# data-man-34/HHFM

Measured on AMD Instinct MI355X. Metric: scored (user,ctx,item) triples/sec + HR@10, Frappe-shape, 1/2/4/8 MI355X, higher is better.
Workload: dtype f32; 1 GPU; FM k=64 Frappe-shape per-row scoring (configs[1], HBM-roofline variant: 8M users + 8M items + 12 ctx ids); rows_per_gpu=33554432, fields=5, k=64, table_rows=16777228, table_bytes=4294970368, parallelism=rows sharded x1, no collective

## Files before the change

hhfm_amd/csrc/fm_rows.hip:

```cpp
#include "hhfm_common.h"

namespace hhfm {

#ifndef HHFM_K1_CAP
#define HHFM_K1_CAP 64
#endif
#ifndef HHFM_K1_WMAP
#define HHFM_K1_WMAP 0
#endif
#ifndef HHFM_K1_CTXKO
#define HHFM_K1_CTXKO 0
#endif
#if (HHFM_K1_WMAP || HHFM_K1_CTXKO) && !defined(HHFM_DIAG_BUILD)
#error "K1 knock-out macros give wrong results: diagnostic builds only (-DHHFM_DIAG_BUILD)"
#endif
#ifndef HHFM_K1_U5
#define HHFM_K1_U5 5
#endif
template <int F>
struct RowsPerLane {
  static constexpr int value =
      F <= 3 ? 6 : (F == 4 ? 4 : (F == 5 ? HHFM_K1_U5 : (F <= 8 ? 3 : 2)));
};

template <int F, int U, bool NT = false>
HHFM_DEV void load_ids(int32_t (&id)[U][F], const int32_t* __restrict__ idx,
                       int64_t base, int64_t B, int g, int RPW, int ncols) {
#pragma unroll
  for (int u = 0; u < U; ++u) {
    int64_t row = base + (int64_t)u * RPW + g;
    const int32_t* p = idx + (row < B ? row : 0) * (int64_t)ncols;
#pragma unroll
    for (int f = 0; f < F; ++f) id[u][f] = load_i32<NT>(p + f);
  }
}

template <int F, int LPR, bool BF16, bool HAS_W, int NTM>
__global__ __launch_bounds__(256) void fm_rows_fast(
    const int32_t* __restrict__ idx, int64_t B, const char* __restrict__ E,
    int64_t M, const float* __restrict__ w, float w0, float* __restrict__ out,
    int32_t* __restrict__ status) {
  constexpr int U = RowsPerLane<F>::value;
  constexpr int RPW = kWave / LPR;
  constexpr int RPI = RPW * U;
  constexpr int64_t ROW_BYTES = (int64_t)LPR * 16;
  constexpr bool NT = NTM == 1;
  using C = Chunk<BF16>;

  const int lane = threadIdx.x & (kWave - 1);
  const int sub = lane & (LPR - 1);
  const int g = lane / LPR;
  const int64_t wave = ((int64_t)blockIdx.x * blockDim.x + threadIdx.x) / kWave;
  const int64_t nwave = ((int64_t)gridDim.x * blockDim.x) / kWave;
  const int64_t stride = nwave * RPI;

  int64_t base = wave * RPI;
  int32_t raw[U][F];
  bool bad = false;
  if (base < B) load_ids<F, U, NT>(raw, idx, base, B, g, RPW, F);

  for (; base < B; base += stride) {
    C c[U][F];
    int32_t id[U][F];
#pragma unroll
    for (int u = 0; u < U; ++u)
#pragma unroll
      for (int f = 0; f < F; ++f) {
        id[u][f] = clamp_id(raw[u][f], M);
        bad |= id[u][f] != raw[u][f];
        if (HHFM_K1_CTXKO && f >= 2) {
#pragma unroll
          for (int e = 0; e < C::kElems; ++e) c[u][f].v[e] = 0.f;
        } else if (NTM == 2 && f < 2)
          c[u][f].template load<true>(E + (int64_t)id[u][f] * ROW_BYTES + sub * 16);
        else
          c[u][f].template load<NT>(E + (int64_t)id[u][f] * ROW_BYTES + sub * 16);
      }

    float wv[U];
    if constexpr (HAS_W) {
      constexpr int WPL = (F + LPR - 1) / LPR;
#pragma unroll
      for (int u = 0; u < U; ++u) {
        wv[u] = 0.f;
#pragma unroll
        for (int r = 0; r < WPL; ++r) {
          const int fsel = r * LPR + sub;
          int32_t my = id[u][0];
#pragma unroll
          for (int f = 1; f < F; ++f) my = (fsel == f) ? id[u][f] : my;
          const float wl = HHFM_K1_WMAP == 1   ? w[my & 0x3ffff]
                           : HHFM_K1_WMAP == 2 ? w[(int64_t)my * 32]
                                               : w[my];
          wv[u] += (fsel < F) ? wl : 0.f;
        }
      }
    }

    load_ids<F, U, NT>(raw, idx, base + stride, B, g, RPW, F);

#pragma unroll
    for (int u = 0; u < U; ++u) {
      float t = 0.f;
#pragma unroll
      for (int e = 0; e < C::kElems; ++e) {
        float s = c[u][0].v[e];
        float q = c[u][0].v[e] * c[u][0].v[e];
#pragma unroll
        for (int f = 1; f < F; ++f) {
          s += c[u][f].v[e];
          q += c[u][f].v[e] * c[u][f].v[e];
        }
        t += 0.5f * (s * s - q);
      }
      t = group_sum<LPR>(t);
      float fb = 0.f;
      if constexpr (HAS_W) fb = group_sum<LPR>(wv[u]);
      const int64_t row = base + (int64_t)u * RPW + g;
      if (sub == 0 && row < B) {
        if constexpr (NT) __builtin_nontemporal_store((t + fb) + w0, out + row);
        else out[row] = (t + fb) + w0;
      }
    }
  }
  report_bad_id(status, bad);
}

template <bool BF16>
__global__ __launch_bounds__(256) void fm_rows_generic(
    const int32_t* __restrict__ idx, int64_t B, int F, const char* __restrict__ E,
    int64_t M, int k, const float* __restrict__ w, float w0,
    float* __restrict__ out, int32_t* __restrict__ status) {
  const int lane = threadIdx.x & (kWave - 1);
  const int64_t wave = ((int64_t)blockIdx.x * blockDim.x + threadIdx.x) / kWave;
  const int64_t nwave = ((int64_t)gridDim.x * blockDim.x) / kWave;
  const int esz = BF16 ? 2 : 4;
  bool bad = false;
  for (int64_t row = wave; row < B; row += nwave) {
    const int32_t* p = idx + row * (int64_t)F;
    for (int f = lane; f < F; f += kWave) bad |= clamp_id(p[f], M) != p[f];
    float t = 0.f;
    for (int e = lane; e < k; e += kWave) {
      float s = 0.f, q = 0.f;
      for (int f = 0; f < F; ++f) {
        const char* r = E + (int64_t)clamp_id(p[f], M) * k * esz;
        float v = BF16 ? bf16_to_f32(reinterpret_cast<const uint16_t*>(r)[e])
                       : reinterpret_cast<const float*>(r)[e];
        s += v;
        q += v * v;
      }
      t += 0.5f * (s * s - q);
    }
    t = group_sum<kWave>(t);
    float fb = 0.f;
    if (w != nullptr)
      for (int f = 0; f < F; ++f) fb += w[clamp_id(p[f], M)];
    if (lane == 0) out[row] = (t + fb) + w0;
  }
  report_bad_id(status, bad);
}

template <int F, int LPR, bool BF16>
__global__ __launch_bounds__(256) void hybrid_rows_fast(
    const int32_t* __restrict__ idx, int64_t B, int nctx,
    const char* __restrict__ E, int64_t M, float* __restrict__ out,
    int32_t* __restrict__ status) {
  constexpr int U = RowsPerLane<F>::value;
  constexpr int RPW = kWave / LPR;
  constexpr int RPI = RPW * U;
  constexpr int64_t ROW_BYTES = (int64_t)LPR * 16;
  using C = Chunk<BF16>;

  const int lane = threadIdx.x & (kWave - 1);
  const int sub = lane & (LPR - 1);
  const int g = lane / LPR;
  const int64_t wave = ((int64_t)blockIdx.x * blockDim.x + threadIdx.x) / kWave;
  const int64_t nwave = ((int64_t)gridDim.x * blockDim.x) / kWave;
  const int64_t stride = nwave * RPI;
  const int ctx_end = 2 + nctx;

  int64_t base = wave * RPI;
  int32_t raw[U][F];
  bool bad = false;
  if (base < B) load_ids<F, U>(raw, idx, base, B, g, RPW, F);

  for (; base < B; base += stride) {
    C c[U][F];
    int32_t id[U][F];
#pragma unroll
    for (int u = 0; u < U; ++u)
#pragma unroll
      for (int f = 0; f < F; ++f) {
        id[u][f] = clamp_id(raw[u][f], M);
        bad |= id[u][f] != raw[u][f];
        c[u][f].load(E + (int64_t)id[u][f] * ROW_BYTES + sub * 16);
      }

    load_ids<F, U>(raw, idx, base + stride, B, g, RPW, F);

#pragma unroll
    for (int u = 0; u < U; ++u) {
      float t = 0.f;
#pragma unroll
      for (int e = 0; e < C::kElems; ++e) {
        float ctx = 0.f, tim = 0.f;
#pragma unroll
        for (int f = 2; f < F; ++f) {
          if (f < ctx_end) ctx += c[u][f].v[e];
          else tim += c[u][f].v[e];
        }
        float h = c[u][0].v[e];
        if (nctx > 0) h = h + ctx;
        if (ctx_end < F) h = h + tim;
        t += h * c[u][1].v[e];
      }
      t = group_sum<LPR>(t);
      const int64_t row = base + (int64_t)u * RPW + g;
      if (sub == 0 && row < B) out[row] = t;
    }
  }
  report_bad_id(status, bad);
}

template <bool BF16>
__global__ __launch_bounds__(256) void hybrid_rows_generic(
    const int32_t* __restrict__ idx, int64_t B, int ncols, int ucol, int icol,
    int c0, int c1, int t0, int t1, const char* __restrict__ E, int64_t M,
    int k, float* __restrict__ out, int32_t* __restrict__ status) {
  const int lane = threadIdx.x & (kWave - 1);
  const int64_t wave = ((int64_t)blockIdx.x * blockDim.x + threadIdx.x) / kWave;
  const int64_t nwave = ((int64_t)gridDim.x * blockDim.x) / kWave;
  const int esz = BF16 ? 2 : 4;
  auto val = [&](int32_t id, int e) -> float {
    const char* r = E + (int64_t)clamp_id(id, M) * k * esz;
    return BF16 ? bf16_to_f32(reinterpret_cast<const uint16_t*>(r)[e])
                : reinterpret_cast<const float*>(r)[e];
  };
  bool bad = false;
  for (int64_t row = wave; row < B; row += nwave) {
    const int32_t* p = idx + row * (int64_t)ncols;
    for (int c = lane; c < ncols; c += kWave)
      if (c == ucol || c == icol || (c >= c0 && c < c1) || (c >= t0 && c < t1))
        bad |= clamp_id(p[c], M) != p[c];
    float t = 0.f;
    for (int e = lane; e < k; e += kWave) {
      float h = val(p[ucol], e);
      if (c1 > c0) {
        float s = 0.f;
        for (int c = c0; c < c1; ++c) s += val(p[c], e);
        h = h + s;
      }
      if (t1 > t0) {
        float s = 0.f;
        for (int c = t0; c < t1; ++c) s += val(p[c], e);
        h = h + s;
      }
      t += h * val(p[icol], e);
    }
    t = group_sum<kWave>(t);
    if (lane == 0) out[row] = t;
  }
  report_bad_id(status, bad);
}

static int grid_for(int64_t rows, int64_t rows_per_block) {
  int64_t g = (rows + rows_per_block - 1) / rows_per_block;
  const int64_t cap = 256 * HHFM_K1_CAP;
  if (g > cap) g = cap;
  if (g < 1) g = 1;
  return (int)g;
}

template <int F, int LPR, bool BF16>
static void launch_fm_fast(const int32_t* idx, int64_t B, const char* E,
                           int64_t M, const float* w, float w0, float* out,
                           bool nt, int32_t* status, hipStream_t s) {
  constexpr int RPB = 4 * (kWave / LPR) * RowsPerLane<F>::value;
  const int grid = grid_for(B, RPB);
  const bool big = M * (int64_t)LPR * 16 >= ((int64_t)1 << 30);
  if (w && nt)
    hipLaunchKernelGGL((fm_rows_fast<F, LPR, BF16, true, 1>), dim3(grid),
                       dim3(256), 0, s, idx, B, E, M, w, w0, out, status);
  else if (w && big && F >= 2)
    hipLaunchKernelGGL((fm_rows_fast<F, LPR, BF16, true, 2>), dim3(grid),
                       dim3(256), 0, s, idx, B, E, M, w, w0, out, status);
  else if (w)
    hipLaunchKernelGGL((fm_rows_fast<F, LPR, BF16, true, 0>), dim3(grid),
                       dim3(256), 0, s, idx, B, E, M, w, w0, out, status);
  else
    hipLaunchKernelGGL((fm_rows_fast<F, LPR, BF16, false, 0>), dim3(grid),
                       dim3(256), 0, s, idx, B, E, M, w, w0, out, status);
}

template <int F, int LPR, bool BF16>
static void launch_hybrid_fast(const int32_t* idx, int64_t B, int nctx,
                               const char* E, int64_t M, float* out,
                               int32_t* status, hipStream_t s) {
  constexpr int RPB = 4 * (kWave / LPR) * RowsPerLane<F>::value;
  const int grid = grid_for(B, RPB);
  hipLaunchKernelGGL((hybrid_rows_fast<F, LPR, BF16>), dim3(grid), dim3(256), 0,
                     s, idx, B, nctx, E, M, out, status);
}

#define HHFM_LPR_SWITCH(LAUNCH, F, BF16, ...)            \
  switch (lpr) {                                         \
    case 4: LAUNCH<F, 4, BF16>(__VA_ARGS__); break;      \
    case 8: LAUNCH<F, 8, BF16>(__VA_ARGS__); break;      \
    case 16: LAUNCH<F, 16, BF16>(__VA_ARGS__); break;    \
    case 32: LAUNCH<F, 32, BF16>(__VA_ARGS__); break;    \
    case 64: LAUNCH<F, 64, BF16>(__VA_ARGS__); break;    \
    default: return false;                               \
  }

#define HHFM_F_SWITCH(LAUNCH, BF16, ...)                          \
  switch (F) {                                                    \
    case 2: HHFM_LPR_SWITCH(LAUNCH, 2, BF16, __VA_ARGS__) break;   \
    case 3: HHFM_LPR_SWITCH(LAUNCH, 3, BF16, __VA_ARGS__) break;   \
    case 4: HHFM_LPR_SWITCH(LAUNCH, 4, BF16, __VA_ARGS__) break;   \
    case 5: HHFM_LPR_SWITCH(LAUNCH, 5, BF16, __VA_ARGS__) break;   \
    case 6: HHFM_LPR_SWITCH(LAUNCH, 6, BF16, __VA_ARGS__) break;   \
    case 7: HHFM_LPR_SWITCH(LAUNCH, 7, BF16, __VA_ARGS__) break;   \
    case 8: HHFM_LPR_SWITCH(LAUNCH, 8, BF16, __VA_ARGS__) break;   \
    case 10: HHFM_LPR_SWITCH(LAUNCH, 10, BF16, __VA_ARGS__) break; \
    case 12: HHFM_LPR_SWITCH(LAUNCH, 12, BF16, __VA_ARGS__) break; \
    default: return false;                                        \
  }

static bool try_fm_fast(const int32_t* idx, int64_t B, int F, const char* E,
                        int64_t M, int lpr, bool bf16, const float* w, float w0,
                        float* out, bool nt, int32_t* status, hipStream_t s) {
  if (bf16) {
    HHFM_F_SWITCH(launch_fm_fast, true, idx, B, E, M, w, w0, out, nt, status, s)
  } else {
    HHFM_F_SWITCH(launch_fm_fast, false, idx, B, E, M, w, w0, out, nt, status, s)
  }
  return true;
}

static bool try_hybrid_fast(const int32_t* idx, int64_t B, int F, int nctx,
                            const char* E, int64_t M, int lpr, bool bf16,
                            float* out, int32_t* status, hipStream_t s) {
  if (bf16) {
    HHFM_F_SWITCH(launch_hybrid_fast, true, idx, B, nctx, E, M, out, status, s)
  } else {
    HHFM_F_SWITCH(launch_hybrid_fast, false, idx, B, nctx, E, M, out, status, s)
  }
  return true;
}

static int lpr_for(int64_t k, int dtype) {
  const int64_t row_bytes = k * (dtype == HHFM_BF16 ? 2 : 4);
  if (row_bytes % 16) return 0;
  return (int)(row_bytes / 16);
}

}

using namespace hhfm;

extern "C" int hhfm_fm_score_rows_ex(const int32_t* idx, int64_t B, int32_t F,
                                     const void* E, int64_t features_M, int32_t k,
                                     int32_t dtype, const float* w, float w0,
                                     float* out, int32_t flags, int32_t* status,
                                     void* stream) {
  if (B < 0 || F < 1 || F > 64 || k < 1 || features_M < 1) return HHFM_EINVAL;
  if (dtype != HHFM_F32 && dtype != HHFM_BF16) return HHFM_EINVAL;
  if (flags & ~HHFM_FLAG_STREAM_TABLE) return HHFM_EINVAL;
  if (B == 0) return HHFM_OK;
  if (!idx || !E || !out) return HHFM_EINVAL;
  hipStream_t s = reinterpret_cast<hipStream_t>(stream);
  const bool bf16 = dtype == HHFM_BF16;
  const int lpr = lpr_for(k, dtype);
  const bool aligned = (reinterpret_cast<uintptr_t>(E) & 15) == 0;
  if (!(lpr && aligned &&
        try_fm_fast(idx, B, F, reinterpret_cast<const char*>(E), features_M,
                    lpr, bf16, w, w0, out, (flags & HHFM_FLAG_STREAM_TABLE) != 0, status,
                    s))) {
    const int grid = grid_for(B, 4);
    if (bf16)
      hipLaunchKernelGGL(fm_rows_generic<true>, dim3(grid), dim3(256), 0, s, idx,
                         B, F, reinterpret_cast<const char*>(E), features_M, k,
                         w, w0, out, status);
    else
      hipLaunchKernelGGL(fm_rows_generic<false>, dim3(grid), dim3(256), 0, s,
                         idx, B, F, reinterpret_cast<const char*>(E),
                         features_M, k, w, w0, out, status);
  }
  return (int)hipGetLastError();
}

extern "C" int hhfm_fm_score_rows(const int32_t* idx, int64_t B, int32_t F,
                                  const void* E, int64_t features_M, int32_t k,
                                  int32_t dtype, const float* w, float w0,
                                  float* out, void* stream) {
  return hhfm_fm_score_rows_ex(idx, B, F, E, features_M, k, dtype, w, w0, out,
                               HHFM_FM_ROWS_DEFAULT_FLAGS, nullptr, stream);
}

extern "C" int hhfm_hybrid_score_rows_ex(const int32_t* idx, int64_t B,
                                         int32_t ncols, int32_t user_col,
                                         int32_t item_col, int32_t ctx_begin,
                                         int32_t ctx_end, int32_t time_begin,
                                         int32_t time_end, const void* E,
                                         int64_t features_M, int32_t k,
                                         int32_t dtype, float* out, int32_t* status,
                                         void* stream) {
  if (B < 0 || ncols < 2 || ncols > 64 || k < 1 || features_M < 1)
    return HHFM_EINVAL;
  if (dtype != HHFM_F32 && dtype != HHFM_BF16) return HHFM_EINVAL;
  auto in_range = [&](int c) { return c >= 0 && c < ncols; };
  if (!in_range(user_col) || !in_range(item_col)) return HHFM_EINVAL;
  if (ctx_begin > ctx_end || time_begin > time_end) return HHFM_EINVAL;
  if (ctx_end > ctx_begin && (!in_range(ctx_begin) || ctx_end > ncols))
    return HHFM_EINVAL;
  if (time_end > time_begin && (!in_range(time_begin) || time_end > ncols))
    return HHFM_EINVAL;
  if (B == 0) return HHFM_OK;
  if (!idx || !E || !out) return HHFM_EINVAL;
  hipStream_t s = reinterpret_cast<hipStream_t>(stream);
  const bool bf16 = dtype == HHFM_BF16;
  const int lpr = lpr_for(k, dtype);
  const bool aligned = (reinterpret_cast<uintptr_t>(E) & 15) == 0;
  const int nctx = ctx_end - ctx_begin;
  const int ntime = time_end - time_begin;
  const bool canonical = user_col == 0 && item_col == 1 &&
                         (nctx == 0 || ctx_begin == 2) &&
                         (ntime == 0 || time_begin == 2 + nctx) &&
                         2 + nctx + ntime == ncols;
  if (!(canonical && lpr && aligned &&
        try_hybrid_fast(idx, B, ncols, nctx,
                        reinterpret_cast<const char*>(E), features_M, lpr,
                        bf16, out, status, s))) {
    const int grid = grid_for(B, 4);
    if (bf16)
      hipLaunchKernelGGL(hybrid_rows_generic<true>, dim3(grid), dim3(256), 0, s,
                         idx, B, ncols, user_col, item_col, ctx_begin, ctx_end,
                         time_begin, time_end,
                         reinterpret_cast<const char*>(E), features_M, k, out, status);
    else
      hipLaunchKernelGGL(hybrid_rows_generic<false>, dim3(grid), dim3(256), 0,
                         s, idx, B, ncols, user_col, item_col, ctx_begin,
                         ctx_end, time_begin, time_end,
                         reinterpret_cast<const char*>(E), features_M, k, out, status);
  }
  return (int)hipGetLastError();
}

extern "C" int hhfm_hybrid_score_rows(const int32_t* idx, int64_t B,
                                      int32_t ncols, int32_t user_col,
                                      int32_t item_col, int32_t ctx_begin,
                                      int32_t ctx_end, int32_t time_begin,
                                      int32_t time_end, const void* E,
                                      int64_t features_M, int32_t k,
                                      int32_t dtype, float* out, void* stream) {
  return hhfm_hybrid_score_rows_ex(idx, B, ncols, user_col, item_col, ctx_begin, ctx_end,
                                   time_begin, time_end, E, features_M, k, dtype, out,
                                   nullptr, stream);
}

extern "C" const char* hhfm_error_string(int code) {
  switch (code) {
    case HHFM_OK: return "ok";
    case HHFM_EINVAL: return "invalid argument";
    case HHFM_EUNSUPPORTED: return "unsupported shape";
    case HHFM_EWORKSPACE: return "workspace too small";
    default: return code > 0 ? hipGetErrorString((hipError_t)code) : "unknown error";
  }
}

extern "C" int hhfm_abi_version(void) { return HHFM_ABI_VERSION; }
```

hhfm_amd/csrc/hhfm_common.h:

```cpp
#pragma once
#include <hip/hip_runtime.h>
#include <stdint.h>

#include <atomic>

#include "../../include/hhfm.h"

#define HHFM_DEV __device__ __forceinline__

namespace hhfm {

constexpr int kWave = 64;

typedef float f32x4_t __attribute__((ext_vector_type(4)));
typedef uint32_t u32x4_t __attribute__((ext_vector_type(4)));

template <bool NT>
HHFM_DEV u32x4_t load16(const void* p) {
  const u32x4_t* q = reinterpret_cast<const u32x4_t*>(p);
  if constexpr (NT) return __builtin_nontemporal_load(q);
  else return *q;
}

template <bool NT>
HHFM_DEV int32_t load_i32(const int32_t* p) {
  if constexpr (NT) return __builtin_nontemporal_load(p);
  else return *p;
}

template <bool BF16>
struct Chunk;

template <>
struct Chunk<false> {
  static constexpr int kElems = 4;
  float v[4];
  template <bool NT = false>
  HHFM_DEV void load(const void* p) {
    const u32x4_t x = load16<NT>(p);
    v[0] = __uint_as_float(x[0]); v[1] = __uint_as_float(x[1]);
    v[2] = __uint_as_float(x[2]); v[3] = __uint_as_float(x[3]);
  }
};

template <>
struct Chunk<true> {
  static constexpr int kElems = 8;
  float v[8];
  template <bool NT = false>
  HHFM_DEV void load(const void* p) {
    const u32x4_t x = load16<NT>(p);
#pragma unroll
    for (int i = 0; i < 4; ++i) {
      v[2 * i] = __uint_as_float(x[i] << 16);
      v[2 * i + 1] = __uint_as_float(x[i] & 0xffff0000u);
    }
  }
};

HHFM_DEV float bf16_to_f32(uint16_t b) { return __uint_as_float(uint32_t(b) << 16); }

HHFM_DEV int32_t clamp_id(int32_t id, int64_t M) {
  return (uint64_t)(uint32_t)id < (uint64_t)M ? id : 0;
}

HHFM_DEV void report_bad_id(int32_t* status, bool bad) {
  if (status == nullptr) return;
  const uint64_t m = __ballot(bad);
  if (m != 0 && (threadIdx.x & (kWave - 1)) == (unsigned)(__ffsll((long long)m) - 1))
    atomicOr(status, HHFM_STATUS_BAD_ID);
}

int launch_check_query_ids(const int32_t* q, int64_t B, int ncols, int ucol, int c0, int c1,
                           int t0, int t1, int64_t M, int32_t* status, hipStream_t s);

template <int G>
HHFM_DEV float group_sum(float x) {
#pragma unroll
  for (int m = G / 2; m >= 1; m >>= 1) x += __shfl_xor(x, m, kWave);
  return x;
}

inline int stream_cu_count(hipStream_t st) {
  static std::atomic<int> cache[64];
  int dev = 0;
  if (hipStreamGetDevice(st, &dev) != hipSuccess && hipGetDevice(&dev) != hipSuccess) return 256;
  if (dev < 0 || dev >= 64) return 256;
  int c = cache[dev].load(std::memory_order_relaxed);
  if (c <= 0) {
    c = 256;
    (void)hipDeviceGetAttribute(&c, hipDeviceAttributeMultiprocessorCount, dev);
    cache[dev].store(c, std::memory_order_relaxed);
  }
  return c;
}

}
```

hhfm_amd/csrc/pybind_hhfm.cpp:

```cpp
#include <pybind11/pybind11.h>
#include <pybind11/stl.h>

#include <cstdint>
#include <stdexcept>
#include <string>
#include <string_view>
#include <vector>

#include "hhfm.h"

namespace py = pybind11;
using uptr = std::uintptr_t;

template <typename T>
static T* P(uptr p) { return reinterpret_cast<T*>(p); }
template <typename T>
static T* P_(uptr p) { return reinterpret_cast<T*>(p); }

static void check(int rc, const char* what) {
  if (rc == HHFM_OK) return;
  std::string msg = std::string(what) + ": " + hhfm_error_string(rc) +
                    " (code " + std::to_string(rc) + ")";
  if (rc == HHFM_EINVAL || rc == HHFM_EUNSUPPORTED || rc == HHFM_EWORKSPACE)
    throw py::value_error(msg);
  throw std::runtime_error(msg);
}

PYBIND11_MODULE(_hhfm, m) {
  m.doc() = "pybind11 binding of libhhfm (MI355X FM-family scoring kernels)";
  m.attr("ABI_VERSION") = HHFM_ABI_VERSION;
  m.attr("F32") = (int)HHFM_F32;
  m.attr("BF16") = (int)HHFM_BF16;
  m.attr("MODE_FM") = (int)HHFM_MODE_FM;
  m.attr("MODE_HHFM") = (int)HHFM_MODE_HHFM;
  m.attr("PLAN_EXACT_FP32") = HHFM_PLAN_EXACT_FP32;
  m.attr("PLAN_NO_SEED") = HHFM_PLAN_NO_SEED;
  m.attr("PLAN_NO_RING") = HHFM_PLAN_NO_RING;
  m.attr("PLAN_RING_ALT") = HHFM_PLAN_RING_ALT;
  m.attr("PLAN_GEMM") = HHFM_PLAN_GEMM;
  m.attr("PLAN_ROW_FM") = HHFM_PLAN_ROW_FM;
  m.attr("PLAN_UNSTAGED") = HHFM_PLAN_UNSTAGED;
  m.attr("PLAN_UNGROUPED") = HHFM_PLAN_UNGROUPED;
  m.attr("PLAN_NARROW") = HHFM_PLAN_NARROW;
  m.attr("PLAN_PER_FIELD") = HHFM_PLAN_PER_FIELD;
  m.attr("PLAN_ONE_WAVE") = HHFM_PLAN_ONE_WAVE;

  m.def("abi_version", [] { return hhfm_abi_version(); });

  m.def("fm_score_rows",
        [](uptr idx, int64_t B, int F, uptr E, int64_t M, int k, int dtype,
           uptr w, float w0, uptr out, uptr stream) {
          int rc;
          {
            py::gil_scoped_release nogil;
            rc = hhfm_fm_score_rows(P<const int32_t>(idx), B, F, P<const void>(E),
                                    M, k, dtype, P<const float>(w), w0,
                                    P<float>(out), P<void>(stream));
          }
          check(rc, "hhfm_fm_score_rows");
        });

  m.def("fm_score_rows_ex",
        [](uptr idx, int64_t B, int F, uptr E, int64_t M, int k, int dtype,
           uptr w, float w0, uptr out, int flags, uptr status, uptr stream) {
          int rc;
          {
            py::gil_scoped_release nogil;
            rc = hhfm_fm_score_rows_ex(P<const int32_t>(idx), B, F, P<const void>(E),
                                       M, k, dtype, P<const float>(w), w0,
                                       P<float>(out), flags, P<int32_t>(status),
                                       P<void>(stream));
          }
          check(rc, "hhfm_fm_score_rows_ex");
        });

  m.def("hybrid_score_rows",
        [](uptr idx, int64_t B, int ncols, int ucol, int icol, int c0, int c1,
           int t0, int t1, uptr E, int64_t M, int k, int dtype, uptr out,
           uptr status, uptr stream) {
          int rc;
          {
            py::gil_scoped_release nogil;
            rc = hhfm_hybrid_score_rows_ex(P<const int32_t>(idx), B, ncols, ucol,
                                           icol, c0, c1, t0, t1, P<const void>(E),
                                           M, k, dtype, P<float>(out), P<int32_t>(status),
                                           P<void>(stream));
          }
          check(rc, "hhfm_hybrid_score_rows_ex");
        });

  m.def("catalog_topk_workspace",
        [](int64_t B, int item_count, int k, int K) {
          size_t ws = 0;
          check(hhfm_catalog_topk_workspace(B, item_count, k, K, &ws),
                "hhfm_catalog_topk_workspace");
          return ws;
        });

  m.def("catalog_topk",
        [](uptr qidx, int64_t B, int ncols, int mode, int ucol, int c0, int c1,
           int t0, int t1, uptr E, int64_t M, int k, int dtype, uptr w,
           int item_row_begin, int item_count, int global_item_base, int K,
           uptr top_score, uptr top_idx, uptr ws, size_t ws_bytes, int plan, uptr status,
           uptr stream) {
          int rc;
          {
            py::gil_scoped_release nogil;
            rc = hhfm_catalog_topk_ex(
                P<const int32_t>(qidx), B, ncols, mode, ucol, c0, c1, t0, t1,
                P<const void>(E), M, k, dtype, P<const float>(w),
                item_row_begin, item_count, global_item_base, K,
                P<float>(top_score), P<int32_t>(top_idx), P<void>(ws), ws_bytes, plan,
                P<int32_t>(status), P<void>(stream));
          }
          check(rc, "hhfm_catalog_topk_ex");
        });

  m.def("check_ids", [](uptr idx, int64_t n, int64_t M, uptr status, uptr stream) {
    int rc;
    {
      py::gil_scoped_release nogil;
      rc = hhfm_check_ids(P<const int32_t>(idx), n, M, P<int32_t>(status), P<void>(stream));
    }
    check(rc, "hhfm_check_ids");
  });

  m.def("status_read", [](uptr status, uptr stream) {
    int rc;
    {
      py::gil_scoped_release nogil;
      rc = hhfm_status_read(P<int32_t>(status), P<void>(stream));
    }
    if (rc != HHFM_OK && rc != HHFM_EINVAL) check(rc, "hhfm_status_read");
    return rc;
  });

  m.def("probe_stream_read", [](uptr buf, int64_t bytes, int mode, uptr sink, uptr stream) {
    int rc;
    {
      py::gil_scoped_release nogil;
      rc = hhfm_probe_stream_read(P<const void>(buf), bytes, mode, P<float>(sink),
                                  P<void>(stream));
    }
    check(rc, "hhfm_probe_stream_read");
  });

  m.def("pf_contains",
        [](uptr keys, int64_t nkeys, int key_cols, uptr codes, int64_t ncodes, uptr rows,
           int64_t B, int ncols, int item_col, uptr cand, int num, uptr out, uptr stream) {
          int rc;
          {
            py::gil_scoped_release nogil;
            rc = hhfm_pf_contains(P<const int32_t>(keys), nkeys, key_cols, P<const int64_t>(codes),
                                  ncodes, P<const int32_t>(rows), B, ncols, item_col,
                                  P<const int32_t>(cand), num, P<uint8_t>(out), P<void>(stream));
          }
          check(rc, "hhfm_pf_contains");
        });

  m.def("topk_walk",
        [](uptr pred, int64_t B, int Pn, uptr target, uptr positive, int TopK, uptr outcome,
           uptr stream) {
          int rc;
          {
            py::gil_scoped_release nogil;
            rc = hhfm_topk_walk(P<const int32_t>(pred), B, Pn, P<const int32_t>(target),
                                P<const uint8_t>(positive), TopK, P<int32_t>(outcome),
                                P<void>(stream));
          }
          check(rc, "hhfm_topk_walk");
        });

  m.def("sample_negative_workspace", [](int64_t B, int num) {
    size_t n = 0;
    check(hhfm_sample_negative_workspace(B, num, &n), "hhfm_sample_negative_workspace");
    return n;
  });

  m.def("sample_negative_workspace_ex", [](int64_t B, int num, int64_t lo, int64_t hi,
                                          int64_t nkeys) {
    size_t n = 0;
    check(hhfm_sample_negative_workspace_ex(B, num, lo, hi, nkeys, &n),
          "hhfm_sample_negative_workspace_ex");
    return n;
  });

  m.def("sample_negative",
// ... 325 lines not shown
```

include/hhfm.h:

```cpp
#ifndef HHFM_H_
#define HHFM_H_

#include <stddef.h>
#include <stdint.h>

#ifdef __cplusplus
extern "C" {
#endif

#define HHFM_ABI_VERSION 6
#define HHFM_CATALOG_WS_ZERO 16384

enum hhfm_dtype { HHFM_F32 = 0, HHFM_BF16 = 1 };

#define HHFM_PLAN_DEFAULT 0
#define HHFM_PLAN_EXACT_FP32 (1 << 0)
#define HHFM_PLAN_NO_SEED (1 << 1)
#define HHFM_PLAN_NO_RING (1 << 2)
#define HHFM_PLAN_RING_ALT (1 << 3)
#define HHFM_PLAN_GEMM (1 << 4)
#define HHFM_PLAN_ROW_FM (1 << 5)
#define HHFM_PLAN_UNSTAGED (1 << 6)
#define HHFM_PLAN_UNGROUPED (1 << 7)
#define HHFM_PLAN_NARROW (1 << 8)
#define HHFM_PLAN_PER_FIELD (1 << 9)
#define HHFM_PLAN_ONE_WAVE (1 << 10)
#define HHFM_PLAN_WIDE_3X4 (1 << 11)
#define HHFM_PLAN_WIDE_2X4 (2 << 11)
#define HHFM_PLAN_WIDE_1X4 (3 << 11)
#define HHFM_PLAN_WIDE_MASK (3 << 11)
#define HHFM_PLAN_STORE (1 << 13)
#define HHFM_PLAN_FUSED (1 << 14)
#define HHFM_PLAN_ALL ((1 << 15) - 1)

enum hhfm_catalog_mode {
  HHFM_MODE_FM = 0,
  HHFM_MODE_HHFM = 1
};

enum hhfm_status {
  HHFM_OK = 0,
  HHFM_EINVAL = -1,
  HHFM_EUNSUPPORTED = -2,
  HHFM_EWORKSPACE = -3
};

const char* hhfm_error_string(int code);
int hhfm_abi_version(void);

int hhfm_fm_score_rows(const int32_t* idx, int64_t B, int32_t F,
                       const void* E, int64_t features_M, int32_t k,
                       int32_t dtype, const float* w, float w0, float* out,
                       void* stream);

#define HHFM_FLAG_STREAM_TABLE 1
#define HHFM_FM_ROWS_DEFAULT_FLAGS 0
#define HHFM_STATUS_BAD_ID 1
int hhfm_fm_score_rows_ex(const int32_t* idx, int64_t B, int32_t F,
                          const void* E, int64_t features_M, int32_t k,
                          int32_t dtype, const float* w, float w0, float* out,
                          int32_t flags, int32_t* status, void* stream);

int hhfm_hybrid_score_rows(const int32_t* idx, int64_t B, int32_t ncols,
                           int32_t user_col, int32_t item_col,
                           int32_t ctx_begin, int32_t ctx_end,
                           int32_t time_begin, int32_t time_end,
                           const void* E, int64_t features_M, int32_t k,
                           int32_t dtype, float* out, void* stream);
int hhfm_hybrid_score_rows_ex(const int32_t* idx, int64_t B, int32_t ncols,
                              int32_t user_col, int32_t item_col,
                              int32_t ctx_begin, int32_t ctx_end,
                              int32_t time_begin, int32_t time_end,
                              const void* E, int64_t features_M, int32_t k,
                              int32_t dtype, float* out, int32_t* status,
                              void* stream);

int hhfm_catalog_topk_workspace(int64_t B, int32_t item_count, int32_t k,
                                int32_t K, size_t* ws_bytes);

int hhfm_catalog_topk(const int32_t* qidx, int64_t B, int32_t ncols,
                      int32_t mode, int32_t user_col, int32_t ctx_begin,
                      int32_t ctx_end, int32_t time_begin, int32_t time_end,
                      const void* E, int64_t features_M, int32_t k,
                      int32_t dtype, const float* w, int32_t item_row_begin,
                      int32_t item_count, int32_t global_item_base, int32_t K,
                      float* top_score, int32_t* top_idx, void* workspace,
                      size_t ws_bytes, void* stream);
int hhfm_catalog_topk_ex(const int32_t* qidx, int64_t B, int32_t ncols,
                         int32_t mode, int32_t user_col, int32_t ctx_begin,
                         int32_t ctx_end, int32_t time_begin, int32_t time_end,
                         const void* E, int64_t features_M, int32_t k,
                         int32_t dtype, const float* w, int32_t item_row_begin,
                         int32_t item_count, int32_t global_item_base, int32_t K,
                         float* top_score, int32_t* top_idx, void* workspace,
                         size_t ws_bytes, int32_t plan, int32_t* status, void* stream);

int hhfm_topk_merge(const float* in_score, const int32_t* in_idx, int32_t R,
                    int64_t B, int32_t K, float* out_score, int32_t* out_idx,
                    void* stream);
int hhfm_topk_merge_host(const float* in_score, const int32_t* in_idx,
                         int32_t R, int64_t B, int32_t K, float* out_score,
                         int32_t* out_idx);

int hhfm_dfm_forward_workspace(int64_t B, int32_t nlayers, const int32_t* layer_dims,
                               int32_t mlp_dtype, size_t* ws_bytes);

enum hhfm_dfm_proj {
  HHFM_DFM_PROJ_OFF = 0,
  HHFM_DFM_PROJ_ON = 1,
  HHFM_DFM_PROJ_AUTO = 2,
  HHFM_DFM_PROJ_CTX = 3,
  HHFM_DFM_PROJ_ITEM = 4
};
int hhfm_dfm_forward_workspace_ex(int64_t B, int32_t F, int32_t k, int64_t features_M,
                                  int32_t nlayers, const int32_t* layer_dims,
                                  int32_t mlp_dtype, int32_t proj_mode, size_t* ws_bytes);
int hhfm_dfm_forward(const int32_t* idx, int64_t B, int32_t F, const void* E,
                     int64_t features_M, int32_t k, int32_t dtype, const float* w,
                     int32_t nlayers, const int32_t* layer_dims, const void* const* Wt,
                     const float* const* bias, int32_t mlp_dtype, const float* Wp,
                     float bp, float* out, void* workspace, size_t ws_bytes,
                     void* stream);
int hhfm_dfm_forward_ex(const int32_t* idx, int64_t B, int32_t F, const void* E,
                        int64_t features_M, int32_t k, int32_t dtype, const float* w,
                        int32_t nlayers, const int32_t* layer_dims, const void* const* Wt,
                        const float* const* bias, int32_t mlp_dtype, const float* Wp,
                        float bp, float* out, int32_t proj_mode, int32_t plan,
                        void* workspace, size_t ws_bytes, void* stream);

int hhfm_dfm_catalog_topk_workspace(int64_t B, int32_t F, int32_t item_count,
                                    int32_t nlayers, const int32_t* layer_dims,
                                    int32_t mlp_dtype, int64_t chunk_rows,
                                    size_t* ws_bytes);
int hhfm_dfm_catalog_topk_workspace_ex(int64_t B, int32_t F, int32_t k,
                                       int64_t features_M, int32_t item_count,
                                       int32_t nlayers, const int32_t* layer_dims,
                                       int32_t mlp_dtype, int64_t chunk_rows,
                                       int32_t proj_mode, size_t* ws_bytes);
int hhfm_dfm_catalog_topk(const int32_t* qidx, int64_t B, int32_t F, int32_t item_col,
                          const void* E, int64_t features_M, int32_t k, int32_t dtype,
                          const float* w, int32_t nlayers, const int32_t* layer_dims,
                          const void* const* Wt, const float* const* bias,
                          int32_t mlp_dtype, const float* Wp, float bp,
                          int32_t item_row_begin, int32_t item_count,
                          int32_t global_item_base, int32_t K, int64_t chunk_rows,
                          float* top_score, int32_t* top_idx, void* workspace,
                          size_t ws_bytes, void* stream);
int hhfm_dfm_catalog_topk_ex(const int32_t* qidx, int64_t B, int32_t F, int32_t item_col,
                             const void* E, int64_t features_M, int32_t k, int32_t dtype,
                             const float* w, int32_t nlayers, const int32_t* layer_dims,
                             const void* const* Wt, const float* const* bias,
                             int32_t mlp_dtype, const float* Wp, float bp,
                             int32_t item_row_begin, int32_t item_count,
                             int32_t global_item_base, int32_t K, int64_t chunk_rows,
                             float* top_score, int32_t* top_idx, int32_t proj_mode,
                             int32_t plan, void* workspace, size_t ws_bytes, void* stream);

int hhfm_afm_forward_workspace(int64_t B, int32_t F, int32_t A, size_t* ws_bytes);
int hhfm_afm_forward(const int32_t* idx, int64_t B, int32_t F, const void* E,
                     int64_t features_M, int32_t k, int32_t dtype, const float* w, float w0,
                     const float* Wt, const float* att_b, const float* att_p, int32_t A,
                     const float* P, float* out, void* workspace, size_t ws_bytes,
                     void* stream);
int hhfm_afm_forward_ex(const int32_t* idx, int64_t B, int32_t F, const void* E,
                        int64_t features_M, int32_t k, int32_t dtype, const float* w,
                        float w0, const float* Wt, const float* att_b, const float* att_p,
                        int32_t A, const float* P, float* out, int32_t plan,
                        void* workspace, size_t ws_bytes, void* stream);

int hhfm_afm_catalog_topk_workspace(int64_t B, int32_t F, int32_t k, int32_t A,
                                    int32_t item_count, int64_t max_cols,
                                    size_t* ws_bytes);
int hhfm_afm_catalog_topk(const int32_t* qidx, int64_t B, int32_t F, const void* E,
                          int64_t features_M, int32_t k, int32_t dtype, const float* w,
                          const float* Wt, const float* att_b, const float* att_p,
                          int32_t A, const float* P, int32_t item_row_begin,
                          int32_t item_count, int32_t global_item_base, int32_t K,
                          int64_t max_cols, float* top_score, int32_t* top_idx,
                          void* workspace, size_t ws_bytes, void* stream);
int hhfm_afm_catalog_topk_workspace_ex(int64_t B, int32_t F, int32_t k, int32_t A,
                                       int32_t item_count, int64_t max_cols, int32_t plan,
                                       size_t* ws_bytes);
int hhfm_afm_catalog_topk_ex(const int32_t* qidx, int64_t B, int32_t F, const void* E,
                             int64_t features_M, int32_t k, int32_t dtype, const float* w,
                             const float* Wt, const float* att_b, const float* att_p,
                             int32_t A, const float* P, int32_t item_row_begin,
                             int32_t item_count, int32_t global_item_base, int32_t K,
                             int64_t max_cols, float* top_score, int32_t* top_idx,
                             int32_t plan, void* workspace, size_t ws_bytes, void* stream);

size_t hhfm_train_workspace(int64_t features_M, int32_t k);
int hhfm_fm_train_step(const int32_t* idx, const float* y, int64_t B, int32_t F, float* E,
                       float* w, float* w0, int64_t features_M, int32_t k, float lr,
                       float lambda_l2, int32_t optimizer, float* accE, float* accw,
                       float* accw0, void* workspace, size_t ws_bytes, float* loss,
                       void* stream);
int hhfm_hhfm_train_step(const int32_t* X, const int32_t* Neg, int64_t B, int32_t ncols,
                         int32_t ctx_begin, int32_t ctx_end, int32_t time_begin,
                         int32_t time_end, int32_t NG, float* E, int64_t features_M,
                         int32_t k, float lr, float lambda_l2, int32_t optimizer, float* accE,
                         void* workspace, size_t ws_bytes, float* loss, void* stream);

int hhfm_dfm_train_workspace(int64_t B, int32_t F, int32_t k, int64_t features_M,
                             int32_t nlayers, const int32_t* layer_dims, size_t* ws_bytes);
int hhfm_dfm_train_state_bytes(int32_t F, int32_t k, int64_t features_M, int32_t nlayers,
                               const int32_t* layer_dims, size_t* state_bytes);
int hhfm_dfm_train_step(const int32_t* idx, const float* y, int64_t B, int32_t F, float* E,
                        float* w, int64_t features_M, int32_t k, int32_t nlayers,
// ... 56 lines not shown
```

Measured before the change: 8.487 billion triples/s.

## Stage hot tail rows of embedding table in LDS for context fields

```diff
diff --git a/hhfm_amd/csrc/fm_rows.hip b/hhfm_amd/csrc/fm_rows.hip
--- a/hhfm_amd/csrc/fm_rows.hip
+++ b/hhfm_amd/csrc/fm_rows.hip
@@ -121,6 +121,229 @@
         if constexpr (NT) __builtin_nontemporal_store((t + fb) + w0, out + row);
         else out[row] = (t + fb) + w0;
       }
+    }
+  }
+  report_bad_id(status, bad);
+}
+
+#ifndef HHFM_K1_HOT_U
+#define HHFM_K1_HOT_U 6
+#endif
+#ifndef HHFM_K1_HOT_CAP
+#define HHFM_K1_HOT_CAP HHFM_K1_CAP
+#endif
+#ifndef HHFM_K1_HOT_AUTO
+#define HHFM_K1_HOT_AUTO 1
+#endif
+constexpr int kHotWindowBytes = 16384;
+
+template <int F>
+struct HotRows {
+  static constexpr int U = F <= 6 ? HHFM_K1_HOT_U : 4;
+  static constexpr int UG = F <= 5 ? 3 : 2;
+};
+
+template <int F, int U, int UG>
+HHFM_DEV void load_ids_slots(int32_t (&id)[UG][F], const int32_t* __restrict__ idx,
+                             int64_t base, int u0, int64_t B, int g, int RPW) {
+#pragma unroll
+  for (int u = 0; u < UG; ++u) {
+    int64_t row = base + (int64_t)(u0 + u) * RPW + g;
+    const int32_t* p = idx + ((u0 + u < U && row < B) ? row : 0) * (int64_t)F;
+#pragma unroll
+    for (int f = 0; f < F; ++f) id[u][f] = p[f];
+  }
+}
+
+template <int F, typename C>
+HHFM_DEV float fm_chunk_term(const C (&c)[F]) {
+  float t = 0.f;
+#pragma unroll
+  for (int e = 0; e < C::kElems; ++e) {
+    float s = c[0].v[e];
+    float q = c[0].v[e] * c[0].v[e];
+#pragma unroll
+    for (int f = 1; f < F; ++f) {
+      s += c[f].v[e];
+      q += c[f].v[e] * c[f].v[e];
+    }
+    t += 0.5f * (s * s - q);
+  }
+  return t;
+}
+
+template <int F, int LPR, bool BF16, bool HAS_W, bool NT01>
+__global__ __launch_bounds__(256) void fm_rows_fast_hot(
+    const int32_t* __restrict__ idx, int64_t B, const char* __restrict__ E,
+    int64_t M, const float* __restrict__ w, float w0, float* __restrict__ out,
+    int32_t* __restrict__ status) {
+  static_assert(F >= 3 && F <= 10 && LPR >= 4, "fields 2.. pack into 8-bit local indices");
+  constexpr int U = HotRows<F>::U;
+  constexpr int UG = HotRows<F>::UG;
+  constexpr int RPW = kWave / LPR;
+  constexpr int RPI = RPW * U;
+  constexpr int64_t ROW_BYTES = (int64_t)LPR * 16;
+  constexpr int T = kHotWindowBytes / (int)ROW_BYTES;
+  constexpr int NC = F - 2;
+  constexpr int PKW = (NC + 3) / 4;
+  constexpr int WPL = (F + LPR - 1) / LPR;
+  static_assert(T <= 256, "local index is 8 bits");
+  using C = Chunk<BF16>;
+
+  __shared__ u32x4_t hot[T * LPR];
+  __shared__ float hotw[HAS_W ? T : 1];
+
+  const int64_t ws = M > T ? M - T : 0;
+  const int nwin = (int)(M - ws);
+  {
+    const char* src = E + ws * ROW_BYTES;
+    for (int i = threadIdx.x; i < nwin * LPR; i += 256) hot[i] = load16<false>(src + (int64_t)i * 16);
+    if constexpr (HAS_W)
+      for (int i = threadIdx.x; i < nwin; i += 256) hotw[i] = w[ws + i];
+  }
+  __syncthreads();
+  const bool reach = ws <= 0x7fffffff;
+  const int32_t ws32 = reach ? (int32_t)ws : 0;
+  const uint32_t nhit = reach ? (uint32_t)nwin : 0u;
+  const uint32_t nm1 = (uint32_t)nwin - 1u;
+
+  const int lane = threadIdx.x & (kWave - 1);
+  const int sub = lane & (LPR - 1);
+  const int g = lane / LPR;
+  const int64_t wave = ((int64_t)blockIdx.x * blockDim.x + threadIdx.x) / kWave;
+  const int64_t nwave = ((int64_t)gridDim.x * blockDim.x) / kWave;
+  const int64_t stride = nwave * RPI;
+
+  int64_t base = wave * RPI;
+  bool bad = false;
+  {
+    int32_t raw[U][F];
+    if (base < B) load_ids<F, U, false>(raw, idx, base, B, g, RPW, F);
+
+    for (; base < B; base += stride) {
+      int32_t id01[U][2];
+      uint32_t pk[U][PKW];
+      bool miss = false;
+#pragma unroll
+      for (int u = 0; u < U; ++u) {
+#pragma unroll
+        for (int j = 0; j < PKW; ++j) pk[u][j] = 0u;
+        bool m = false;
+#pragma unroll
+        for (int f = 0; f < F; ++f) {
+          const int32_t id = clamp_id(raw[u][f], M);
+          bad |= id != raw[u][f];
+          if (f < 2) {
+            id01[u][f] = id;
+          } else {
+            const uint32_t d = (uint32_t)(id - ws32);
+            m |= d >= nhit;
+            pk[u][(f - 2) >> 2] |= (d < nm1 ? d : nm1) << (8 * ((f - 2) & 3));
+          }
+        }
+        miss |= m && (base + (int64_t)u * RPW + g < B);
+      }
+      if (__ballot(miss) != 0) break;
+
+      C c01[U][2];
+      float wg[U];
+#pragma unroll
+      for (int u = 0; u < U; ++u) {
+#pragma unroll
+        for (int f = 0; f < 2; ++f)
+          c01[u][f].template load<NT01>(E + (int64_t)id01[u][f] * ROW_BYTES + sub * 16);
+      }
+      if constexpr (HAS_W) {
+#pragma unroll
+        for (int u = 0; u < U; ++u) wg[u] = w[sub == 1 ? id01[u][1] : id01[u][0]];
+      }
+
+      load_ids<F, U, false>(raw, idx, base + stride, B, g, RPW, F);
+
+#pragma unroll
+      for (int u = 0; u < U; ++u) {
+        C c[F];
+        c[0] = c01[u][0];
+        c[1] = c01[u][1];
+#pragma unroll
+        for (int f = 2; f < F; ++f) {
+          const uint32_t li = (pk[u][(f - 2) >> 2] >> (8 * ((f - 2) & 3))) & 0xffu;
+          c[f].set(hot[li * LPR + sub]);
+        }
+        float t = group_sum<LPR>(fm_chunk_term<F>(c));
+        float fb = 0.f;
+        if constexpr (HAS_W) {
+          float wv = 0.f;
+#pragma unroll
+          for (int r = 0; r < WPL; ++r) {
+            const int fsel = r * LPR + sub;
+            int j = fsel - 2;
+            j = j < 0 ? 0 : (j > NC - 1 ? NC - 1 : j);
+            uint32_t word = pk[u][0];
+#pragma unroll
+            for (int q = 1; q < PKW; ++q) word = (j >> 2) == q ? pk[u][q] : word;
+            const float wl = hotw[(word >> (8 * (j & 3))) & 0xffu];
+            wv += (fsel < 2) ? wg[u] : ((fsel < F) ? wl : 0.f);
+          }
+          fb = group_sum<LPR>(wv);
+        }
+        const int64_t row = base + (int64_t)u * RPW + g;
+        if (sub == 0 && row < B) out[row] = (t + fb) + w0;
+      }
+    }
+  }
+
+  if (base < B) {
+    int u0 = 0;
+    int32_t raw[UG][F];
+    load_ids_slots<F, U, UG>(raw, idx, base, u0, B, g, RPW);
+    while (base < B) {
+      C c[UG][F];
+      int32_t id[UG][F];
+#pragma unroll
+      for (int u = 0; u < UG; ++u)
+#pragma unroll
+        for (int f = 0; f < F; ++f) {
+          id[u][f] = clamp_id(raw[u][f], M);
+          bad |= id[u][f] != raw[u][f];
+          if (NT01 && f < 2)
+            c[u][f].template load<true>(E + (int64_t)id[u][f] * ROW_BYTES + sub * 16);
+          else
+            c[u][f].template load<false>(E + (int64_t)id[u][f] * ROW_BYTES + sub * 16);
+        }
+      float wv[UG];
+      if constexpr (HAS_W) {
+#pragma unroll
+        for (int u = 0; u < UG; ++u) {
+          wv[u] = 0.f;
+#pragma unroll
+          for (int r = 0; r < WPL; ++r) {
+            const int fsel = r * LPR + sub;
+            int32_t my = id[u][0];
+#pragma unroll
+            for (int f = 1; f < F; ++f) my = (fsel == f) ? id[u][f] : my;
+            const float wl = w[my];
+            wv[u] += (fsel < F) ? wl : 0.f;
+          }
+        }
+      }
+      int64_t nbase = base;
+      int nu0 = u0 + UG;
+      if (nu0 >= U) {
+        nu0 = 0;
+        nbase += stride;
+      }
+      load_ids_slots<F, U, UG>(raw, idx, nbase, nu0, B, g, RPW);
+#pragma unroll
+      for (int u = 0; u < UG; ++u) {
+        float t = group_sum<LPR>(fm_chunk_term<F>(c[u]));
+        float fb = 0.f;
+        if constexpr (HAS_W) fb = group_sum<LPR>(wv[u]);
+        const int64_t row = base + (int64_t)(u0 + u) * RPW + g;
+        if (sub == 0 && u0 + u < U && row < B) out[row] = (t + fb) + w0;
+      }
+      base = nbase;
+      u0 = nu0;
     }
   }
   report_bad_id(status, bad);
@@ -263,12 +486,36 @@
   report_bad_id(status, bad);
 }
 
-static int grid_for(int64_t rows, int64_t rows_per_block) {
+static int grid_for(int64_t rows, int64_t rows_per_block, hipStream_t s) {
   int64_t g = (rows + rows_per_block - 1) / rows_per_block;
-  const int64_t cap = 256 * HHFM_K1_CAP;
+  const int64_t cap = (int64_t)stream_cu_count(s) * HHFM_K1_CAP;
   if (g > cap) g = cap;
   if (g < 1) g = 1;
   return (int)g;
+}
+
+template <int F, int LPR, bool BF16>
+static bool launch_fm_hot(const int32_t* idx, int64_t B, const char* E,
+                          int64_t M, const float* w, float w0, float* out,
+                          bool forced, int32_t* status, hipStream_t s) {
+  constexpr int RPB = 4 * (kWave / LPR) * HotRows<F>::U;
+  const int64_t blocks = (B + RPB - 1) / RPB;
+  const int64_t cap = (int64_t)stream_cu_count(s) * HHFM_K1_HOT_CAP;
+  if (blocks < cap && !forced) return false;
+  int64_t g = blocks >= cap ? cap : blocks / 4;
+  if (g < 1) g = 1;
+  const int grid = (int)g;
+  const bool big = M * (int64_t)LPR * 16 >= ((int64_t)1 << 30);
+  if (w && big)
+    hipLaunchKernelGGL((fm_rows_fast_hot<F, LPR, BF16, true, true>), dim3(grid),
+                       dim3(256), 0, s, idx, B, E, M, w, w0, out, status);
+  else if (w)
+    hipLaunchKernelGGL((fm_rows_fast_hot<F, LPR, BF16, true, false>), dim3(grid),
+                       dim3(256), 0, s, idx, B, E, M, w, w0, out, status);
+  else
+    hipLaunchKernelGGL((fm_rows_fast_hot<F, LPR, BF16, false, false>), dim3(grid),
+                       dim3(256), 0, s, idx, B, E, M, w, w0, out, status);
+  return true;
 }
 
 template <int F, int LPR, bool BF16>
@@ -276,7 +523,7 @@
                            int64_t M, const float* w, float w0, float* out,
                            bool nt, int32_t* status, hipStream_t s) {
   constexpr int RPB = 4 * (kWave / LPR) * RowsPerLane<F>::value;
-  const int grid = grid_for(B, RPB);
+  const int grid = grid_for(B, RPB, s);
   const bool big = M * (int64_t)LPR * 16 >= ((int64_t)1 << 30);
   if (w && nt)
     hipLaunchKernelGGL((fm_rows_fast<F, LPR, BF16, true, 1>), dim3(grid),
@@ -297,7 +544,7 @@
                                const char* E, int64_t M, float* out,
                                int32_t* status, hipStream_t s) {
   constexpr int RPB = 4 * (kWave / LPR) * RowsPerLane<F>::value;
-  const int grid = grid_for(B, RPB);
+  const int grid = grid_for(B, RPB, s);
   hipLaunchKernelGGL((hybrid_rows_fast<F, LPR, BF16>), dim3(grid), dim3(256), 0,
                      s, idx, B, nctx, E, M, out, status);
 }
@@ -337,6 +584,28 @@
   return true;
 }
 
+#define HHFM_F_SWITCH_HOT(BF16, ...)                                            \
+  switch (F) {                                                                 \
+    case 3: HHFM_LPR_SWITCH(return launch_fm_hot, 3, BF16, __VA_ARGS__) break; \
+    case 4: HHFM_LPR_SWITCH(return launch_fm_hot, 4, BF16, __VA_ARGS__) break; \
+    case 5: HHFM_LPR_SWITCH(return launch_fm_hot, 5, BF16, __VA_ARGS__) break; \
+    case 6: HHFM_LPR_SWITCH(return launch_fm_hot, 6, BF16, __VA_ARGS__) break; \
+    case 7: HHFM_LPR_SWITCH(return launch_fm_hot, 7, BF16, __VA_ARGS__) break; \
+    case 8: HHFM_LPR_SWITCH(return launch_fm_hot, 8, BF16, __VA_ARGS__) break; \
+    default: return false;                                                     \
+  }
+
+static bool try_fm_hot(const int32_t* idx, int64_t B, int F, const char* E,
+                       int64_t M, int lpr, bool bf16, const float* w, float w0,
+                       float* out, bool forced, int32_t* status, hipStream_t s) {
+  if (bf16) {
+    HHFM_F_SWITCH_HOT(true, idx, B, E, M, w, w0, out, forced, status, s)
+  } else {
+    HHFM_F_SWITCH_HOT(false, idx, B, E, M, w, w0, out, forced, status, s)
+  }
+  return false;
+}
+
 static bool try_hybrid_fast(const int32_t* idx, int64_t B, int F, int nctx,
                             const char* E, int64_t M, int lpr, bool bf16,
                             float* out, int32_t* status, hipStream_t s) {
@@ -365,18 +634,29 @@
                                      void* stream) {
   if (B < 0 || F < 1 || F > 64 || k < 1 || features_M < 1) return HHFM_EINVAL;
   if (dtype != HHFM_F32 && dtype != HHFM_BF16) return HHFM_EINVAL;
-  if (flags & ~HHFM_FLAG_STREAM_TABLE) return HHFM_EINVAL;
+  if (flags & ~(HHFM_FLAG_STREAM_TABLE | HHFM_FLAG_HOT_TAIL | HHFM_FLAG_NO_HOT_TAIL))
+    return HHFM_EINVAL;
+  const bool hot_forced = (flags & HHFM_FLAG_HOT_TAIL) != 0;
+  if (hot_forced && (flags & (HHFM_FLAG_NO_HOT_TAIL | HHFM_FLAG_STREAM_TABLE))) return HHFM_EINVAL;
   if (B == 0) return HHFM_OK;
   if (!idx || !E || !out) return HHFM_EINVAL;
   hipStream_t s = reinterpret_cast<hipStream_t>(stream);
   const bool bf16 = dtype == HHFM_BF16;
   const int lpr = lpr_for(k, dtype);
   const bool aligned = (reinterpret_cast<uintptr_t>(E) & 15) == 0;
+  if (HHFM_K1_HOT_AUTO || hot_forced) {
+    const bool allowed = !(flags & (HHFM_FLAG_NO_HOT_TAIL | HHFM_FLAG_STREAM_TABLE));
+    if (allowed && lpr && aligned &&
+        try_fm_hot(idx, B, F, reinterpret_cast<const char*>(E), features_M, lpr, bf16, w, w0,
+                   out, hot_forced, status, s))
+      return (int)hipGetLastError();
+    if (hot_forced) return HHFM_EUNSUPPORTED;
+  }
   if (!(lpr && aligned &&
         try_fm_fast(idx, B, F, reinterpret_cast<const char*>(E), features_M,
                     lpr, bf16, w, w0, out, (flags & HHFM_FLAG_STREAM_TABLE) != 0, status,
                     s))) {
-    const int grid = grid_for(B, 4);
+    const int grid = grid_for(B, 4, s);
     if (bf16)
       hipLaunchKernelGGL(fm_rows_generic<true>, dim3(grid), dim3(256), 0, s, idx,
                          B, F, reinterpret_cast<const char*>(E), features_M, k,
@@ -431,7 +711,7 @@
         try_hybrid_fast(idx, B, ncols, nctx,
                         reinterpret_cast<const char*>(E), features_M, lpr,
                         bf16, out, status, s))) {
-    const int grid = grid_for(B, 4);
+    const int grid = grid_for(B, 4, s);
     if (bf16)
       hipLaunchKernelGGL(hybrid_rows_generic<true>, dim3(grid), dim3(256), 0, s,
                          idx, B, ncols, user_col, item_col, ctx_begin, ctx_end,
diff --git a/hhfm_amd/csrc/hhfm_common.h b/hhfm_amd/csrc/hhfm_common.h
--- a/hhfm_amd/csrc/hhfm_common.h
+++ b/hhfm_amd/csrc/hhfm_common.h
@@ -35,27 +35,27 @@
 struct Chunk<false> {
   static constexpr int kElems = 4;
   float v[4];
-  template <bool NT = false>
-  HHFM_DEV void load(const void* p) {
-    const u32x4_t x = load16<NT>(p);
+  HHFM_DEV void set(const u32x4_t x) {
     v[0] = __uint_as_float(x[0]); v[1] = __uint_as_float(x[1]);
     v[2] = __uint_as_float(x[2]); v[3] = __uint_as_float(x[3]);
   }
+  template <bool NT = false>
+  HHFM_DEV void load(const void* p) { set(load16<NT>(p)); }
 };
 
 template <>
 struct Chunk<true> {
   static constexpr int kElems = 8;
   float v[8];
-  template <bool NT = false>
-  HHFM_DEV void load(const void* p) {
-    const u32x4_t x = load16<NT>(p);
+  HHFM_DEV void set(const u32x4_t x) {
 #pragma unroll
     for (int i = 0; i < 4; ++i) {
       v[2 * i] = __uint_as_float(x[i] << 16);
       v[2 * i + 1] = __uint_as_float(x[i] & 0xffff0000u);
     }
   }
+  template <bool NT = false>
+  HHFM_DEV void load(const void* p) { set(load16<NT>(p)); }
 };
 
 HHFM_DEV float bf16_to_f32(uint16_t b) { return __uint_as_float(uint32_t(b) << 16); }
diff --git a/hhfm_amd/csrc/pybind_hhfm.cpp b/hhfm_amd/csrc/pybind_hhfm.cpp
--- a/hhfm_amd/csrc/pybind_hhfm.cpp
+++ b/hhfm_amd/csrc/pybind_hhfm.cpp
@@ -33,6 +33,9 @@
   m.attr("BF16") = (int)HHFM_BF16;
   m.attr("MODE_FM") = (int)HHFM_MODE_FM;
   m.attr("MODE_HHFM") = (int)HHFM_MODE_HHFM;
+  m.attr("FLAG_STREAM_TABLE") = HHFM_FLAG_STREAM_TABLE;
+  m.attr("FLAG_HOT_TAIL") = HHFM_FLAG_HOT_TAIL;
+  m.attr("FLAG_NO_HOT_TAIL") = HHFM_FLAG_NO_HOT_TAIL;
   m.attr("PLAN_EXACT_FP32") = HHFM_PLAN_EXACT_FP32;
   m.attr("PLAN_NO_SEED") = HHFM_PLAN_NO_SEED;
   m.attr("PLAN_NO_RING") = HHFM_PLAN_NO_RING;
diff --git a/include/hhfm.h b/include/hhfm.h
--- a/include/hhfm.h
+++ b/include/hhfm.h
@@ -54,6 +54,8 @@
                        void* stream);
 
 #define HHFM_FLAG_STREAM_TABLE 1
+#define HHFM_FLAG_HOT_TAIL 2
+#define HHFM_FLAG_NO_HOT_TAIL 4
 #define HHFM_FM_ROWS_DEFAULT_FLAGS 0
 #define HHFM_STATUS_BAD_ID 1
 int hhfm_fm_score_rows_ex(const int32_t* idx, int64_t B, int32_t F,
```

Result: faster. 9.265 billion triples/s, median of 6 (+9.2%).
